# yc015/fully-automated-multi-heartbeat-echocardiography-video-segmentation-and-motion-tracking

Hardware: AMD Instinct MI355X
Metric: 32f×112×112 clips/sec at 1/2/4/8 MI355X; Dice Δ vs CPU ref (higher is better)
Workload: dtype fp32

## Files before the change

### fully-automated-multi-heartbeat-echocardiography-video-segmentation-and-motion-tracking_amd/csrc/wino4_common.h

```cpp
#pragma once
#include "common.h"

typedef float f32x2 __attribute__((ext_vector_type(2)));

struct W4Geo {
  int TR, TC;
  int TH, TW;
  int RP;
  int SS;
  int RS;
  int NI;
  int n_cob;
  int gpr;
  FastDiv fd_cob, fd_gpr, fd_th, fd_tc, fd_rp, fd_ss;
#ifdef CLASFV_KNOCKOUTS
  int stagger, stagger_groups;
#endif
};

namespace {

constexpr int W4_WAVES = 4;
constexpr int W4_THREADS = 64 * W4_WAVES;
constexpr int W4_NU = 14;
template <int DPW>
struct W4Ring {
  static constexpr int STAGE = W4_WAVES * DPW * 1024;
  static constexpr int NR = DPW == 4 ? 4 : 3;
  static constexpr int STEP = NR - 2;
  static constexpr int LDS = NR * STAGE + 1024;
};
constexpr int W4_CS = 20;
constexpr int W4_ZS = 16 * W4_CS + 4;
constexpr int W4_ZBYTES = 42 * W4_ZS * 4;
static_assert(W4_ZBYTES <= W4Ring<4>::LDS && W4Ring<4>::LDS <= 80 * 1024 && W4Ring<5>::LDS <= 80 * 1024 &&
                  W4Ring<6>::LDS <= 80 * 1024,
              "two blocks per CU");

__device__ inline int xcd_swizzle4(int b, int nb) {
  const int q = nb >> 3, r = nb & 7, x = b & 7, i = b >> 3;
  return (x < r ? x * (q + 1) : r * (q + 1) + (x - r) * q) + i;
}

constexpr int vm_wait(int n) { return (n & 0xF) | ((n >> 4) << 14) | 0x0F70; }


template <int RH>
__device__ inline void bt_rows(const f32x2 (&e)[5], f32x2 (&t)[3]) {
  if constexpr (RH == 0) {
    t[0] = e[0] * 4.f - e[2] * 5.f + e[4];
    const f32x2 s = e[1] + e[2], u = e[3] + e[4], d = e[1] - e[2], w = e[4] - e[3];
    t[1] = u - s * 4.f;
    t[2] = w + d * 4.f;
  } else {
    const f32x2 x = e[3] - e[1], y = e[2] - e[0];
    t[0] = x + y * 2.f;
    t[1] = x - y * 2.f;
    t[2] = e[0] * 4.f - e[2] * 5.f + e[4];
  }
}

template <int CH>
__device__ inline void bt_cols(const f32x2 (&t)[6], f32x2 (&v)[3]) {
  if constexpr (CH == 0) {
    v[0] = t[0] * 4.f - t[2] * 5.f + t[4];
    const f32x2 s = t[1] + t[2], u = t[3] + t[4], d = t[1] - t[2], w = t[4] - t[3];
    v[1] = u - s * 4.f;
    v[2] = w + d * 4.f;
  } else {
    const f32x2 x = t[4] - t[2], y = t[3] - t[1];
    v[0] = x + y * 2.f;
    v[1] = x - y * 2.f;
    v[2] = t[1] * 4.f - t[3] * 5.f + t[5];
  }
}

inline bool wino4_geometry(const ConvParams& p, W4Geo* g, int* n_blocks, int cob_w = 48, int fill16 = 0) {
#ifdef CLASFV_KNOCKOUTS
  g->stagger = 0;
  g->stagger_groups = 1;
#endif
  if (p.Cout % cob_w || p.Cin % 8) return false;
  const int TH = (p.Ho + 3) / 4, TW = (p.Wo + 3) / 4;
  const long rows = (long)p.N * p.To * TH;
  auto tr_for = [&](int tc) {
    for (int d = 16 / tc; d >= 1; --d)
      if (((long)p.To * TH) % d == 0) return d;
    return 1;
  };
  auto pitch = [&](int TR, int TC) {
    const int PC = 4 * TC + 2, rp0 = (PC - 1) + (PC - 1) / 4 + 1;
    int best = 1 << 30;
    for (int rp = rp0; rp < rp0 + 16; ++rp)
      for (int ss = 6 * rp; ss < 6 * rp + 16; ++ss) {
        const int ni = (2 * TR * ss + 63) / 64;
        if (ni > W4_WAVES * 6) continue;
        int cnt[16] = {0}, m = 0;
        for (int t = 0; t < TR * TC; ++t) {
          const int v = ((t / TC) * ss + 5 * (t % TC)) & 15;
          if (++cnt[v] > m) m = cnt[v];
        }
        const int score = m * 1000 + (ni <= 16 ? 0 : 100) + ni;
        if (score < best) best = score, g->RP = rp, g->SS = ss;
      }
    return best != (1 << 30);
  };
  int TC = 0;
  for (int d = TW < 16 ? TW : 16; d >= 1 && !TC; --d)
    if (TW % d == 0) TC = d;
  int TR = tr_for(TC);
  if (fill16) {
    int bc = TC, br = TR;
    for (int d = TW < 16 ? TW : 16; d >= fill16; --d)
      if (TW % d == 0 && tr_for(d) * d > br * bc) bc = d, br = tr_for(d);
    if ((bc != TC || br != TR) && br * bc >= 12 && pitch(br, bc)) TC = bc, TR = br;
  }
  if (TR * TC < 12 || !pitch(TR, TC)) return false;
  g->TR = TR, g->TC = TC, g->TH = TH, g->TW = TW;
  g->RS = TR * g->SS;
  g->NI = (2 * g->RS + 63) / 64;
  g->n_cob = p.Cout / cob_w;
  g->gpr = TW / TC;
  g->fd_cob = fast_div(g->n_cob);
  g->fd_gpr = fast_div(g->gpr);
  g->fd_th = fast_div(TH);
  g->fd_tc = fast_div(TC);
  g->fd_rp = fast_div(g->RP);
  g->fd_ss = fast_div(g->SS);
  *n_blocks = (int)(rows / TR) * g->gpr * g->n_cob;
  return true;
}

}
```

### fully-automated-multi-heartbeat-echocardiography-video-segmentation-and-motion-tracking_amd/csrc/winograd4w.hip

```cpp
#include <cstdio>
#include <cstdlib>
#include <type_traits>

#include "wino4_common.h"

namespace {

template <int NTN>
struct W4W {
  static constexpr int NV = 18 * NTN;
  static constexpr int UQ = NTN == 9 ? 14 : 9;
  static constexpr int NU = (NV + 4 * UQ - 1) / (4 * UQ) * UQ;
};

constexpr int W4W_ZT = 20;
constexpr int W4W_ZP = 16 * W4W_ZT + 4;
constexpr int W4W_ZBUF = 42 * W4W_ZP;

constexpr int W4W_NTA = 7;
__device__ inline void mfma_v(f32x4& c, float a, float b) {
  asm volatile("s_nop 1\n\tv_mfma_f32_16x16x4_f32 %0, %1, %2, %0" : "+v"(c) : "v"(a), "v"(b));
}
__device__ inline void w4w_drain() { asm volatile("s_nop 7\n\ts_nop 4" ::: "memory"); }

// ... 166 lines not shown
      if constexpr ((KO & 2) == 0) {
        const int gn = gi + UQ;
        u[gi % UQ] = gn < NU ? load_u(k, gn) : load_u(k + 1, gn - NU);
      }
    }
    constexpr int NB = (NTN < W4W_NTA ? NTN : W4W_NTA) * 18, FG = NB / 4, RM = NB % 4;
#pragma unroll
    for (int gi = 0; gi < NU; ++gi) {
      if (gi < FG)
        __builtin_amdgcn_sched_group_barrier(0x008, 4, 0);
      else if (gi == FG && RM)
        __builtin_amdgcn_sched_group_barrier(0x008, RM, 0);
      if constexpr ((KO & 2) == 0) __builtin_amdgcn_sched_group_barrier(0x020, 1, 0);
    }
  } while (++k < nchunk);
  if constexpr (NTN > W4W_NTA) w4w_drain();
  __builtin_amdgcn_s_waitcnt(vm_wait(0));
  __syncthreads();
#ifdef CLASFV_KNOCKOUTS
  if constexpr ((KO & 512) != 0) st_[2] = __builtin_amdgcn_s_memrealtime();
#endif

  if constexpr ((KO & 4) != 0) {
    float sum = 0.f;
#pragma unroll
    for (int nt = 0; nt < NTN; ++nt)
#pragma unroll
      for (int r = 0; r < 3; ++r)
#pragma unroll
        for (int jj = 0; jj < 3; ++jj) sum += acc[nt][r][jj][0] + acc[nt][r][jj][3];
    if (sum == 1234.5f) reinterpret_cast<float*>(p.y)[tid] = sum;
    return;
  }
  float* Z0 = reinterpret_cast<float*>(smem);
  const int q = lane >> 4, l16 = lane & 15;
  const size_t plane = (size_t)p.N * p.To * H * W * 8;
  float* yout = reinterpret_cast<float*>(p.y);
  const int ub = tid & 3, ucq = (tid >> 2) & 3, utile = tid >> 4;
  const int useg = fdiv(utile, g.fd_tc), utc = utile - useg * g.TC;
  const int uR = R0 + useg, uf = fdiv(uR, g.fd_th), uty = uR - uf * g.TH;
  const int uxx = 4 * (tx0 + utc) + ub;
  const bool ulive = utile < NT && uxx < W;
  const int eb = ub == 3 ? 1 : ub;
  const int CO = p.Cout;
  auto write_planes = [&](int nt) __attribute__((always_inline)) {
    float* Z = Z0 + (nt & 1) * W4W_ZBUF;
    if (ch == 0) {
#pragma unroll
      for (int r = 0; r < 3; ++r) {
        const f32x4 m0 = acc[nt][r][0], m1 = acc[nt][r][1], m2 = acc[nt][r][2];
        f32x4* zp = reinterpret_cast<f32x4*>(Z + ((3 * rh + r) * 3) * W4W_ZP + l16 * W4W_ZT + 4 * q);
        zp[0] = m0 + m1 + m2;
        zp[W4W_ZP / 4] = psub4(m1, m2);
        zp[2 * W4W_ZP / 4] = m1 + m2;
      }
    } else {
#pragma unroll
      for (int r = 0; r < 3; ++r) {
        const f32x4 m0 = acc[nt][r][0], m1 = acc[nt][r][1], m2 = acc[nt][r][2];
        f32x4* zp = reinterpret_cast<f32x4*>(Z + (18 + (3 * rh + r) * 4) * W4W_ZP + l16 * W4W_ZT + 4 * q);
        const f32x4 sm = m0 + m1, df = psub4(m0, m1);
        zp[0] = sm;
        zp[W4W_ZP / 4] = 2.f * df;
        zp[2 * W4W_ZP / 4] = 4.f * sm;
        zp[3 * W4W_ZP / 4] = 8.f * df + m2;
      }
    }
  };
  auto read_unit = [&](int nt, f32x4 (&P)[6]) __attribute__((always_inline)) {
    const float* Z = Z0 + (nt & 1) * W4W_ZBUF;
#pragma unroll
    for (int i = 0; i < 6; ++i)
      P[i] = *reinterpret_cast<const f32x4*>(Z + (i * 3 + eb) * W4W_ZP + utile * W4W_ZT + 4 * ucq) +
             *reinterpret_cast<const f32x4*>(Z + (18 + i * 4 + ub) * W4W_ZP + utile * W4W_ZT + 4 * ucq);
  };
  const int co0 = cob * NTN * 16 + 4 * ucq;
  const size_t upix = (size_t)(uf * H + 4 * uty) * W + uxx;
  float* ybase[4];
#pragma unroll
  for (int aa = 0; aa < 4; ++aa) {
    const size_t px = upix + (size_t)aa * W;
    ybase[aa] = yout + (C8 ? (size_t)(co0 >> 3) * plane + px * 8 + (co0 & 7) : px * CO + co0);
  }
  const size_t nt_step = C8 ? 2 * plane : 16;
  f32x4 biasv[NTN];
#pragma unroll
  for (int nt = 0; nt < NTN; ++nt)
    biasv[nt] = p.bias ? *reinterpret_cast<const f32x4*>(p.bias + co0 + nt * 16) : f32x4{0.f, 0.f, 0.f, 0.f};
  auto store_unit = [&](int nt, const f32x4 (&P)[6]) __attribute__((always_inline)) {
    const f32x4 bias = biasv[nt];
    const f32x4 s12 = P[1] + P[2], d12 = psub4(P[1], P[2]), s34 = P[3] + P[4], d34 = psub4(P[3], P[4]);
    f32x4 y[4];
    y[0] = P[0] + s12 + s34;
    y[1] = d12 + 2.f * d34;
    y[2] = s12 + 4.f * s34;
    y[3] = d12 + 8.f * d34 + P[5];
#pragma unroll
    for (int aa = 0; aa < 4; ++aa) {
      if (4 * uty + aa >= H) break;
      f32x4 o = y[aa] + bias;
      if constexpr (RELU) {
#pragma unroll
        for (int c = 0; c < 4; ++c) o[c] = relu1(o[c]);
      }
      float* dst = ybase[aa] + nt * nt_step;
      if constexpr ((KO & 128) != 0) {
        if (o[0] == 1234.5f) *reinterpret_cast<f32x4*>(dst) = o;
      } else {
        *reinterpret_cast<f32x4*>(dst) = o;
      }
    }
  };
  if constexpr ((KO & 256) != 0) {
#pragma unroll
    for (int nt = 0; nt < NTN; ++nt) {
      __builtin_amdgcn_sched_barrier(0);
      write_planes(nt);
      __syncthreads();
      if (ulive) {
        f32x4 P[6];
        read_unit(nt, P);
        store_unit(nt, P);
      }
    }
  } else {
    write_planes(0);
#pragma unroll
    for (int nt = 0; nt < NTN; ++nt) {
      __builtin_amdgcn_sched_barrier(0);
      __syncthreads();
      f32x4 P[6];
      if (ulive) read_unit(nt, P);
      if (nt + 1 < NTN) write_planes(nt + 1);
      if (ulive) store_unit(nt, P);
    }
  }
#ifdef CLASFV_KNOCKOUTS
  if constexpr ((KO & 512) != 0) {
    __builtin_amdgcn_s_waitcnt(0);
    __syncthreads();
    st_[3] = __builtin_amdgcn_s_memrealtime();
    if (tid == 0 && blockIdx.x < W4W_NSTAMP) {
      unsigned long long* o = g_w4w_stamps[blockIdx.x];
      o[0] = st_[0], o[1] = st_[1], o[2] = st_[2], o[3] = st_[3];
      o[8] = __builtin_amdgcn_s_getreg((4 << 0) | (0 << 6) | (31 << 11));
      o[9] = __builtin_amdgcn_s_getreg((20 << 0) | (0 << 6) | (31 << 11));
    }
  }
#endif
}

constexpr int W4R_WAVES = 12;
constexpr int W4R_THREADS = 64 * W4R_WAVES;
constexpr int W4R_DPW = 2;
constexpr int W4R_STAGE = W4R_WAVES * W4R_DPW * 1024;
constexpr int W4R_NR = 4;
constexpr int W4R_NZ = 3;
constexpr int W4R_LDS = W4R_NZ * W4W_ZBUF * 4;
static_assert(W4R_LDS >= W4R_NR * W4R_STAGE + 1024 && W4R_LDS <= 160 * 1024, "ring and planes fit LDS");

template <int NTN>
struct W4R {
  static constexpr int NV = 6 * NTN;
  static constexpr int UQ = NTN == 9 ? 7 : NTN == 5 ? 8 : 9;
  static constexpr int NU = (NV + 4 * UQ - 1) / (4 * UQ) * UQ;
};

template <int RH, int R>
__device__ inline f32x2 bt_row(const f32x2 (&e)[5]) {
  if constexpr (RH == 0) {
    if constexpr (R == 0) {
      return e[0] * 4.f - e[2] * 5.f + e[4];
    } else if constexpr (R == 1) {
      const f32x2 s = e[1] + e[2], u = e[3] + e[4];
      return u - s * 4.f;
    } else {
      const f32x2 d = e[1] - e[2], w = e[4] - e[3];
      return w + d * 4.f;
    }
  } else {
    if constexpr (R == 2) {
      return e[0] * 4.f - e[2] * 5.f + e[4];
    } else {
      const f32x2 x = e[3] - e[1], y = e[2] - e[0];
      if constexpr (R == 0)
        return x + y * 2.f;
      else
        return x - y * 2.f;
    }
  }
}

template <int NTN, bool C8, int KO = 0, bool RELU = true, int NR = W4R_NR, int CPB = 1, bool NTS = false>
__global__ __launch_bounds__(W4R_THREADS) __attribute__((amdgpu_waves_per_eu(3, 3))) void conv_wino4r(ConvParams p,
                                                                                                       W4Geo g) {
  using WR = W4R<NTN>;
  constexpr int STAGE = W4R_STAGE, UQ = WR::UQ, NU = WR::NU, NV = WR::NV;
  constexpr int STEP = NR / 2;
  static_assert(NR * STAGE + 1024 <= W4R_LDS, "ring fits the plane buffers' LDS");
  __shared__ __align__(16) char smem[W4R_LDS];
  char* sink = smem + NR * STAGE;

#ifdef CLASFV_KNOCKOUTS
  unsigned long long st_[4] = {0, 0, 0, 0};
  if constexpr ((KO & 512) != 0) st_[0] = __builtin_amdgcn_s_memrealtime();
#endif
#ifdef CLASFV_KNOCKOUTS
  if (g.stagger > 0 && blockIdx.x < 256) {
    const int sg = (blockIdx.x >> 3) % g.stagger_groups;
    if (sg) {
      const unsigned long long t0 = __builtin_amdgcn_s_memrealtime(), dt = (unsigned long long)sg * g.stagger;
      while (__builtin_amdgcn_s_memrealtime() - t0 < dt) __builtin_amdgcn_s_sleep(8);
    }
  }
#endif
  const __amdgpu_buffer_rsrc_t xr = __builtin_amdgcn_make_buffer_rsrc(
      const_cast<void*>(p.x), (short)0, (int)((size_t)p.N * p.Ti * p.Hi * p.Wi * p.Cin * 4), 0x00020000);
  const int tid = threadIdx.x, lane = tid & 63;
  const int wid = __builtin_amdgcn_readfirstlane(tid >> 6);
  const int blk = xcd_swizzle4(blockIdx.x, gridDim.x);
  const int grp = fdiv(blk, g.fd_cob), cob = blk - grp * g.n_cob;
  const int rg = fdiv(grp, g.fd_gpr), gx = grp - rg * g.gpr;
  const int R0 = rg * g.TR, tx0 = gx * g.TC;
  const int H = p.Ho, W = p.Wo, C = p.Cin;
  const int nchunk = C >> 3;
  const int NT = g.TR * g.TC;
  const int wq = wid / 3, r = wid - 3 * wq, rh = wq >> 1, ch = wq & 1;

  unsigned d_off[W4R_DPW];
#pragma unroll
  for (int j = 0; j < W4R_DPW; ++j) {
    const int ins = wid + W4R_WAVES * j, s = ins * 64 + lane;
    unsigned off = 0x80000000u;
    if (ins < g.NI && s < 2 * g.RS) {
      const int hf = s >= g.RS ? 1 : 0, sl = s - hf * g.RS;
      const int seg = fdiv(sl, g.fd_ss), ss = sl - seg * g.SS;
      const int rr = fdiv(ss, g.fd_rp), cs = ss - rr * g.RP;
      const int m5 = cs / 5, k5 = cs - 5 * m5, c = 4 * m5 + k5;
      if (rr < 6 && k5 < 4 && c < 4 * g.TC + 2) {
        const int R = R0 + seg, f = fdiv(R, g.fd_th), ty = R - f * g.TH;
        const int yy = 4 * ty - 1 + rr, xx = 4 * tx0 - 1 + c;
        if ((unsigned)yy < (unsigned)H && (unsigned)xx < (unsigned)W) off = (((f * H + yy) * W + xx) * C + hf * 4) * 4;
      }
    }
    d_off[j] = off;
  }
  auto issue_raw = [&](int k, int stage) __attribute__((always_inline)) {
#pragma unroll
    for (int j = 0; j < W4R_DPW; ++j) {
      const int ins = wid + W4R_WAVES * j;
      __builtin_amdgcn_raw_ptr_buffer_load_lds(
          xr, (__attribute__((address_space(3))) void*)(ins < g.NI ? smem + stage * STAGE + ins * 1024 : sink), 16,
          d_off[j], k < nchunk ? k * 32 : 0, 0, 0);
    }
  };

  const int t = lane & 15, k4 = lane >> 4;
  const int tv = t < NT ? t : 0;
  const int tseg = fdiv(tv, g.fd_tc), tcol = tv - tseg * g.TC;
  const int lane_off = ((k4 >> 1) * g.RS + tseg * g.SS + rh * g.RP + 5 * tcol) * 16 + (k4 & 1) * 8;
  const int rp16 = g.RP * 16;
  auto transform = [&](int stage, f32x2 (&a)[3]) __attribute__((always_inline)) {
    if constexpr ((KO & 1) != 0) {
#pragma unroll
      for (int jj = 0; jj < 3; ++jj) a[jj] = f32x2{(float)(lane + jj + stage), (float)(lane - jj)};
      return;
    }
    const char* base = smem + stage * STAGE + lane_off;
    auto body = [&](auto rh_c, auto ch_c, auto r_c) __attribute__((always_inline)) {
      constexpr int RH = decltype(rh_c)::value, CH = decltype(ch_c)::value, RR = decltype(r_c)::value;
      f32x2 tt[6];
      if constexpr (CPB == 0) {
        auto col_read = [&](int c, f32x2 (&e)[5]) __attribute__((always_inline)) {
          const int co = (c + (c >> 2)) * 16;
#pragma unroll
          for (int q = 0; q < 5; ++q) e[q] = *reinterpret_cast<const f32x2*>(base + q * rp16 + co);
        };
        f32x2 e0[5], e1[5];
        col_read(0, e0);
        __builtin_amdgcn_sched_barrier(0);
#pragma unroll
        for (int c = 0; c < 6; c += 2) {
          if (c + 1 < 6) col_read(c + 1, e1);
          tt[c] = bt_row<RH, RR>(e0);
          __builtin_amdgcn_sched_barrier(0);
          if (c + 2 < 6) col_read(c + 2, e0);
          tt[c + 1] = bt_row<RH, RR>(e1);
          __builtin_amdgcn_sched_barrier(0);
        }
      } else {
#pragma unroll
        for (int c = 0; c < 6; ++c) {
          const int co = (c + (c >> 2)) * 16;
          f32x2 e[5];
#pragma unroll
          for (int q = 0; q < 5; ++q) e[q] = *reinterpret_cast<const f32x2*>(base + q * rp16 + co);
          tt[c] = bt_row<RH, RR>(e);
          if (c % CPB == CPB - 1) __builtin_amdgcn_sched_barrier(0);
        }
      }
      bt_cols<CH>(tt, a);
    };
    using I0 = std::integral_constant<int, 0>;
    using I1 = std::integral_constant<int, 1>;
    using I2 = std::integral_constant<int, 2>;
    switch (wid) {
      case 0: body(I0{}, I0{}, I0{}); break;
      case 1: body(I0{}, I0{}, I1{}); break;
      case 2: body(I0{}, I0{}, I2{}); break;
      case 3: body(I0{}, I1{}, I0{}); break;
      case 4: body(I0{}, I1{}, I1{}); break;
      case 5: body(I0{}, I1{}, I2{}); break;
      case 6: body(I1{}, I0{}, I0{}); break;
      case 7: body(I1{}, I0{}, I1{}); break;
      case 8: body(I1{}, I0{}, I2{}); break;
      case 9: body(I1{}, I1{}, I0{}); break;
      case 10: body(I1{}, I1{}, I1{}); break;
      default: body(I1{}, I1{}, I2{}); break;
    }
  };

  const __amdgpu_buffer_rsrc_t ur = __builtin_amdgcn_make_buffer_rsrc(
      const_cast<float*>(reinterpret_cast<const float*>(p.w) + ((size_t)cob * nchunk * W4R_WAVES + wid) * (NU * 256)),
      (short)0, nchunk * W4R_WAVES * NU * 256 * 4, 0x00020000);
  auto load_u = [&](int k, int gi) __attribute__((always_inline)) {
    return __builtin_bit_cast(f32x4, __builtin_amdgcn_raw_buffer_load_b128(
                                         ur, lane * 16, ((k < nchunk ? k : 0) * (W4R_WAVES * NU * 256) + gi * 256) * 4, 0));
  };

  f32x4 acc[NTN][3];
#pragma unroll
  for (int nt = 0; nt < NTN; ++nt)
#pragma unroll
    for (int jj = 0; jj < 3; ++jj) acc[nt][jj] = f32x4{0.f, 0.f, 0.f, 0.f};
  f32x4 u[UQ];
  f32x2 a[3];

#pragma unroll
  for (int d = 0; d < STEP; ++d) {
    issue_raw(d, d);
    __builtin_amdgcn_sched_barrier(0);
  }
#pragma unroll
  for (int gi = 0; gi < UQ; ++gi) u[gi] = load_u(0, gi);
  __builtin_amdgcn_sched_barrier(0);

  int k = 0;
#pragma unroll 1
  do {
    const int ph = k % NR;
    if (ph % STEP == 0) {
      __builtin_amdgcn_s_waitcnt(vm_wait(UQ));
      __builtin_amdgcn_sched_barrier(0);
      if constexpr ((KO & 16) == 0) __builtin_amdgcn_s_barrier();
      __builtin_amdgcn_sched_barrier(0);
#ifdef CLASFV_KNOCKOUTS
      if constexpr ((KO & 512) != 0)
        if (k == 0) st_[1] = __builtin_amdgcn_s_memrealtime();
#endif
      if constexpr ((KO & 8) == 0) {
#pragma unroll
        for (int d = NR - STEP; d < NR; ++d) issue_raw(k + d, (ph + d) % NR);
      }
    }
    __builtin_amdgcn_sched_barrier(0);
    transform(ph, a);
    __builtin_amdgcn_sched_barrier(0);
#pragma unroll
    for (int gi = 0; gi < NU; ++gi) {
#pragma unroll
      for (int c = 0; c < 4; ++c) {
        const int m = 4 * gi + c;
        if (m < NV) {
          const int jj = m % 3, ks = (m / 3) % 2, nt = m / 6;
          acc[nt][jj] = __builtin_amdgcn_mfma_f32_16x16x4f32(u[gi % UQ][c], ks ? a[jj].y : a[jj].x, acc[nt][jj], 0, 0, 0);
        }
      }
      if constexpr ((KO & 2) == 0) {
        const int gn = gi + UQ;
        u[gi % UQ] = gn < NU ? load_u(k, gn) : load_u(k + 1, gn - NU);
      }
    }
    constexpr int FG = NV / 4, RM = NV % 4;
#pragma unroll
    for (int gi = 0; gi < NU; ++gi) {
      if (gi < FG)
        __builtin_amdgcn_sched_group_barrier(0x008, 4, 0);
      else if (gi == FG && RM)
        __builtin_amdgcn_sched_group_barrier(0x008, RM, 0);
      if constexpr ((KO & 2) == 0) __builtin_amdgcn_sched_group_barrier(0x020, 1, 0);
    }
  } while (++k < nchunk);
  __builtin_amdgcn_s_waitcnt(vm_wait(0));
  __syncthreads();
#ifdef CLASFV_KNOCKOUTS
  if constexpr ((KO & 512) != 0) st_[2] = __builtin_amdgcn_s_memrealtime();
#endif

  if constexpr ((KO & 4) != 0) {
    float sum = 0.f;
#pragma unroll
    for (int nt = 0; nt < NTN; ++nt)
#pragma unroll
      for (int jj = 0; jj < 3; ++jj) sum += acc[nt][jj][0] + acc[nt][jj][3];
    if (sum == 1234.5f) reinterpret_cast<float*>(p.y)[tid] = sum;
    return;
  }
  float* Z0 = reinterpret_cast<float*>(smem);
  const int q = lane >> 4, l16 = lane & 15;
  const size_t plane = (size_t)p.N * p.To * H * W * 8;
  float* yout = reinterpret_cast<float*>(p.y);
  const int ug = tid >> 8, ut = tid & 255;
  const int ub = ut & 3, ucq = (ut >> 2) & 3, utile = ut >> 4;
  const int useg = fdiv(utile, g.fd_tc), utc = utile - useg * g.TC;
  const int uR = R0 + useg, uf = fdiv(uR, g.fd_th), uty = uR - uf * g.TH;
  const int uxx = 4 * (tx0 + utc) + ub;
  const bool ulive = utile < NT && uxx < W;
  const int eb = ub == 3 ? 1 : ub;
  const int CO = p.Cout;
  const int zrow = 3 * rh + r;
  auto write_planes = [&](int nt, int buf) __attribute__((always_inline)) {
    float* Z = Z0 + buf * W4W_ZBUF;
    const f32x4 m0 = acc[nt][0], m1 = acc[nt][1], m2 = acc[nt][2];
    if (ch == 0) {
      f32x4* zp = reinterpret_cast<f32x4*>(Z + (zrow * 3) * W4W_ZP + l16 * W4W_ZT + 4 * q);
      zp[0] = m0 + m1 + m2;
      zp[W4W_ZP / 4] = psub4(m1, m2);
      zp[2 * W4W_ZP / 4] = m1 + m2;
    } else {
      f32x4* zp = reinterpret_cast<f32x4*>(Z + (18 + zrow * 4) * W4W_ZP + l16 * W4W_ZT + 4 * q);
      const f32x4 sm = m0 + m1, df = psub4(m0, m1);
      zp[0] = sm;
      zp[W4W_ZP / 4] = 2.f * df;
      zp[2 * W4W_ZP / 4] = 4.f * sm;
      zp[3 * W4W_ZP / 4] = 8.f * df + m2;
    }
  };
  auto read_unit = [&](int buf, f32x4 (&P)[6]) __attribute__((always_inline)) {
    const float* Z = Z0 + buf * W4W_ZBUF;
#pragma unroll
    for (int i = 0; i < 6; ++i)
      P[i] = *reinterpret_cast<const f32x4*>(Z + (i * 3 + eb) * W4W_ZP + utile * W4W_ZT + 4 * ucq) +
             *reinterpret_cast<const f32x4*>(Z + (18 + i * 4 + ub) * W4W_ZP + utile * W4W_ZT + 4 * ucq);
  };
  const int co0 = cob * NTN * 16 + 4 * ucq;
  const size_t upix = (size_t)(uf * H + 4 * uty) * W + uxx;
  float* ybase[4];
#pragma unroll
  for (int aa = 0; aa < 4; ++aa) {
    const size_t px = upix + (size_t)aa * W;
    ybase[aa] = yout + (C8 ? (size_t)(co0 >> 3) * plane + px * 8 + (co0 & 7) : px * CO + co0);
  }
  const size_t nt_step = C8 ? 2 * plane : 16;
  constexpr int NRND = (NTN + W4R_NZ - 1) / W4R_NZ;
  f32x4 biasv[NRND];
#pragma unroll
  for (int rd = 0; rd < NRND; ++rd) {
    const int nt = W4R_NZ * rd + ug;
    biasv[rd] = p.bias && nt < NTN ? *reinterpret_cast<const f32x4*>(p.bias + co0 + nt * 16) : f32x4{0.f, 0.f, 0.f, 0.f};
  }
  auto store_unit = [&](int nt, const f32x4& bias, const f32x4 (&P)[6]) __attribute__((always_inline)) {
    const f32x4 s12 = P[1] + P[2], d12 = psub4(P[1], P[2]), s34 = P[3] + P[4], d34 = psub4(P[3], P[4]);
    f32x4 y[4];
    y[0] = P[0] + s12 + s34;
    y[1] = d12 + 2.f * d34;
    y[2] = s12 + 4.f * s34;
    y[3] = d12 + 8.f * d34 + P[5];
#pragma unroll
    for (int aa = 0; aa < 4; ++aa) {
      if (4 * uty + aa >= H) break;
      f32x4 o = y[aa] + bias;
      if constexpr (RELU) {
#pragma unroll
        for (int c = 0; c < 4; ++c) o[c] = relu1(o[c]);
      }
      float* dst = ybase[aa] + nt * nt_step;
      if constexpr ((KO & 128) != 0) {
        if (o[0] == 1234.5f) *reinterpret_cast<f32x4*>(dst) = o;
      } else if constexpr (NTS || (KO & 2048) != 0) {
        __builtin_nontemporal_store(o, reinterpret_cast<f32x4*>(dst));
      } else {
        *reinterpret_cast<f32x4*>(dst) = o;
      }
    }
  };
#pragma unroll
  for (int b = 0; b < W4R_NZ; ++b)
    if (b < NTN) write_planes(b, b);
#pragma unroll
  for (int rd = 0; rd < NRND; ++rd) {
    __builtin_amdgcn_sched_barrier(0);
    __syncthreads();
    const int nt_u = W4R_NZ * rd + ug;
    const bool live = ulive && nt_u < NTN;
    f32x4 P[6];
    if (live) read_unit(ug, P);
    if (rd + 1 < NRND) {
      __syncthreads();
#pragma unroll
      for (int b = 0; b < W4R_NZ; ++b)
        if (W4R_NZ * (rd + 1) + b < NTN) write_planes(W4R_NZ * (rd + 1) + b, b);
    }
    if (live) store_unit(nt_u, biasv[rd], P);
  }
#ifdef CLASFV_KNOCKOUTS
  if constexpr ((KO & 512) != 0) {
    __builtin_amdgcn_s_waitcnt(0);
    __syncthreads();
    st_[3] = __builtin_amdgcn_s_memrealtime();
    if (tid == 0 && blockIdx.x < W4W_NSTAMP) {
      unsigned long long* o = g_w4w_stamps[blockIdx.x];
      o[0] = st_[0], o[1] = st_[1], o[2] = st_[2], o[3] = st_[3];
      o[8] = __builtin_amdgcn_s_getreg((4 << 0) | (0 << 6) | (31 << 11));
      o[9] = __builtin_amdgcn_s_getreg((20 << 0) | (0 << 6) | (31 << 11));
    }
  }
#endif
}

template <int NTN, int KO = 0, int NR = W4R_NR, int CPB = 1>
hipError_t launch_w4r(const ConvParams& p, const W4Geo& g, int n_blocks, hipStream_t s) {
  const dim3 grid(n_blocks), block(W4R_THREADS);
  if (!(p.vflags & CLASFV_VARIANT_W4R_CACHED_STORES)) {
    if (p.y_c8 && p.relu) {
      CLASFV_LAUNCH((conv_wino4r<NTN, true, KO, true, NR, CPB, true>), grid, block, 0, s, p, g);
      return hipGetLastError();
    }
    if (p.relu) {
      CLASFV_LAUNCH((conv_wino4r<NTN, false, KO, true, NR, CPB, true>), grid, block, 0, s, p, g);
      return hipGetLastError();
    }
  }
  if (p.y_c8 && p.relu)
    CLASFV_LAUNCH((conv_wino4r<NTN, true, KO, true, NR, CPB>), grid, block, 0, s, p, g);
  else if (p.relu)
    CLASFV_LAUNCH((conv_wino4r<NTN, false, KO, true, NR, CPB>), grid, block, 0, s, p, g);
  else if (p.y_c8)
    CLASFV_LAUNCH((conv_wino4r<NTN, true, KO, false, NR, CPB>), grid, block, 0, s, p, g);
  else
    CLASFV_LAUNCH((conv_wino4r<NTN, false, KO, false, NR, CPB>), grid, block, 0, s, p, g);
  return hipGetLastError();
}

constexpr int W4W_FILL = 1;

int wino4w_ntn(int cout) {
  if (cout % 16) return 0;
  for (int n : {9, 6})
    if ((cout / 16) % n == 0) return n;
  return 0;
}

template <int NTN, int DPW, int KO = 0>
hipError_t launch_w4w(const ConvParams& p, const W4Geo& g, int n_blocks, hipStream_t s) {
  const dim3 grid(n_blocks), block(W4_THREADS);
  if (p.y_c8 && p.relu)
    CLASFV_LAUNCH((conv_wino4w<NTN, true, DPW, KO, true>), grid, block, 0, s, p, g);
  else if (p.relu)
    CLASFV_LAUNCH((conv_wino4w<NTN, false, DPW, KO, true>), grid, block, 0, s, p, g);
  else if (p.y_c8)
    CLASFV_LAUNCH((conv_wino4w<NTN, true, DPW, KO, false>), grid, block, 0, s, p, g);
  else
    CLASFV_LAUNCH((conv_wino4w<NTN, false, DPW, KO, false>), grid, block, 0, s, p, g);
  return hipGetLastError();
}

template <int NTN, int KO = 0>
hipError_t launch_w4w_dpw(const ConvParams& p, const W4Geo& g, int n_blocks, hipStream_t s) {
  const int dpw = (g.NI + W4_WAVES - 1) / W4_WAVES;
  return dpw <= 4 ? launch_w4w<NTN, 4, KO>(p, g, n_blocks, s)
                  : dpw == 5 ? launch_w4w<NTN, 5, KO>(p, g, n_blocks, s) : launch_w4w<NTN, 6, KO>(p, g, n_blocks, s);
}

}

bool wino4w_supported(const ConvParams& p) {
  W4Geo g;
  int nb;
  const int ntn = wino4w_ntn(p.Cout);
  return ntn && !p.in_bf16 && !p.out_bf16 && !p.stem && !p.x2 && !p.res && p.KT == 1 && p.KH == 3 && p.KW == 3 &&
         p.sh == 1 && p.sw == 1 && p.st == 1 && p.ph == 1 && p.pw == 1 && p.pt == 0 && p.Ho == p.Hi &&
         p.Wo == p.Wi && p.To == p.Ti &&
         (size_t)p.N * p.To * p.Ho * p.Wo * (p.Cin > p.Cout ? p.Cin : p.Cout) < ((size_t)1 << 31) &&
         wino4_geometry(p, &g, &nb, 16 * ntn, W4W_FILL);
}

hipError_t launch_wino4w(const ConvParams& p, hipStream_t s) {
  if (!wino4w_supported(p)) return hipErrorInvalidValue;
  W4Geo g;
  int nb;
  const int ntn = wino4w_ntn(p.Cout);
  wino4_geometry(p, &g, &nb, 16 * ntn, W4W_FILL);
  return ntn == 9 ? launch_w4w_dpw<9>(p, g, nb, s) : launch_w4w_dpw<6>(p, g, nb, s);
}

double wino4w_exec_gflop(const ConvParams& p) {
  W4Geo g;
  int nb;
  const int ntn = wino4w_ntn(p.Cout);
  return ntn && wino4_geometry(p, &g, &nb, 16 * ntn, W4W_FILL) ? 2.0 * nb * 16.0 * 36.0 * p.Cin * 16.0 * ntn * 1e-9 : 0.0;
}

size_t wino4w_weight_floats(int cin_p, int cout_p) {
  const int ntn = wino4w_ntn(cout_p);
  if (!ntn) return 0;
  const int nu = ntn == 9 ? W4W<9>::NU : W4W<6>::NU;
  return (size_t)(cout_p / (16 * ntn)) * (cin_p / 8) * W4_WAVES * nu * 256;
}

void wino4w_transform_weights(const double* w, int cout, int cin, int cout_p, int cin_p, float* U) {
  static const double G[6][3] = {{1.0 / 4, 0, 0},
                                 {-1.0 / 6, -1.0 / 6, -1.0 / 6},
                                 {-1.0 / 6, 1.0 / 6, -1.0 / 6},
                                 {1.0 / 24, 1.0 / 12, 1.0 / 6},
                                 {1.0 / 24, -1.0 / 12, 1.0 / 6},
                                 {0, 0, 1}};
  const int ntn = wino4w_ntn(cout_p);
  const int nu = ntn == 9 ? W4W<9>::NU : W4W<6>::NU;
  const int nch = cin_p / 8, cw = 16 * ntn;
  const size_t total = wino4w_weight_floats(cin_p, cout_p);
  for (size_t i = 0; i < total; ++i) U[i] = 0.f;
  for (int o = 0; o < cout; ++o)
    for (int c = 0; c < cin; ++c) {
      const double* gw = w + ((size_t)o * cin + c) * 9;
      double tmp[6][3];
      for (int i = 0; i < 6; ++i)
        for (int v = 0; v < 3; ++v) tmp[i][v] = G[i][0] * gw[0 * 3 + v] + G[i][1] * gw[1 * 3 + v] + G[i][2] * gw[2 * 3 + v];
      const int cob = o / cw, nt = (o % cw) / 16, n = o % 16;
      const int chunk = c / 8, k4 = (c % 8) / 2, ks = c % 2;
      for (int i = 0; i < 6; ++i)
        for (int j = 0; j < 6; ++j) {
          const double uu = tmp[i][0] * G[j][0] + tmp[i][1] * G[j][1] + tmp[i][2] * G[j][2];
          const int wv = (i / 3) * 2 + j / 3, r = i % 3, jj = j % 3;
          const int m = ((nt * 3 + r) * 2 + ks) * 3 + jj, gi = m / 4, comp = m % 4;
          U[((((((size_t)cob * nch + chunk) * W4_WAVES + wv) * nu + gi) * 64) + k4 * 16 + n) * 4 + comp] = (float)uu;
        }
    }
}

int wino4r_ntn(int cout) {
  if (cout % 16) return 0;
  for (int n : {9, 6})
    if ((cout / 16) % n == 0) return n;
  return 0;
}

static int w4r_nu(int ntn) { return ntn == 9 ? W4R<9>::NU : ntn == 6 ? W4R<6>::NU : W4R<5>::NU; }

bool wino4r_supported(const ConvParams& p) {
  W4Geo g;
  int nb;
  const int ntn = wino4r_ntn(p.Cout);
  return ntn && !p.in_bf16 && !p.out_bf16 && !p.stem && !p.x2 && !p.res && p.KT == 1 && p.KH == 3 && p.KW == 3 &&
         p.sh == 1 && p.sw == 1 && p.st == 1 && p.ph == 1 && p.pw == 1 && p.pt == 0 && p.Ho == p.Hi &&
         p.Wo == p.Wi && p.To == p.Ti &&
         (size_t)p.N * p.To * p.Ho * p.Wo * (p.Cin > p.Cout ? p.Cin : p.Cout) < ((size_t)1 << 31) &&
         wino4_geometry(p, &g, &nb, 16 * ntn, W4W_FILL);
}

hipError_t launch_wino4r(const ConvParams& p, hipStream_t s) {
  if (!wino4r_supported(p)) return hipErrorInvalidValue;
  W4Geo g;
  int nb;
  const int ntn = wino4r_ntn(p.Cout);
  wino4_geometry(p, &g, &nb, 16 * ntn, W4W_FILL);
  return ntn == 9 ? launch_w4r<9>(p, g, nb, s) : launch_w4r<6>(p, g, nb, s);
}

double wino4r_exec_gflop(const ConvParams& p) {
  W4Geo g;
  int nb;
  const int ntn = wino4r_ntn(p.Cout);
  return ntn && wino4_geometry(p, &g, &nb, 16 * ntn, W4W_FILL) ? 2.0 * nb * 16.0 * 36.0 * p.Cin * 16.0 * ntn * 1e-9 : 0.0;
}

size_t wino4r_weight_floats(int cin_p, int cout_p) {
  const int ntn = wino4r_ntn(cout_p);
  if (!ntn) return 0;
  return (size_t)(cout_p / (16 * ntn)) * (cin_p / 8) * W4R_WAVES * w4r_nu(ntn) * 256;
}

void wino4r_transform_weights(const double* w, int cout, int cin, int cout_p, int cin_p, float* U) {
  static const double G[6][3] = {{1.0 / 4, 0, 0},
                                 {-1.0 / 6, -1.0 / 6, -1.0 / 6},
                                 {-1.0 / 6, 1.0 / 6, -1.0 / 6},
                                 {1.0 / 24, 1.0 / 12, 1.0 / 6},
                                 {1.0 / 24, -1.0 / 12, 1.0 / 6},
                                 {0, 0, 1}};
  const int ntn = wino4r_ntn(cout_p);
  const int nu = w4r_nu(ntn);
  const int nch = cin_p / 8, cw = 16 * ntn;
  const size_t total = wino4r_weight_floats(cin_p, cout_p);
  for (size_t i = 0; i < total; ++i) U[i] = 0.f;
  for (int o = 0; o < cout; ++o)
    for (int c = 0; c < cin; ++c) {
      const double* gw = w + ((size_t)o * cin + c) * 9;
      double tmp[6][3];
      for (int i = 0; i < 6; ++i)
        for (int v = 0; v < 3; ++v) tmp[i][v] = G[i][0] * gw[0 * 3 + v] + G[i][1] * gw[1 * 3 + v] + G[i][2] * gw[2 * 3 + v];
      const int cob = o / cw, nt = (o % cw) / 16, n = o % 16;
      const int chunk = c / 8, k4 = (c % 8) / 2, ks = c % 2;
      for (int i = 0; i < 6; ++i)
        for (int j = 0; j < 6; ++j) {
          const double uu = tmp[i][0] * G[j][0] + tmp[i][1] * G[j][1] + tmp[i][2] * G[j][2];
          const int wv = ((i / 3) * 2 + j / 3) * 3 + i % 3, jj = j % 3;
          const int m = (nt * 2 + ks) * 3 + jj, gi = m / 4, comp = m % 4;
          U[((((((size_t)cob * nch + chunk) * W4R_WAVES + wv) * nu + gi) * 64) + k4 * 16 + n) * 4 + comp] = (float)uu;
        }
    }
}

#ifdef CLASFV_KNOCKOUTS
void wino4w_stamps(unsigned long long* out, int n) {
  (void)hipMemcpyFromSymbol(out, HIP_SYMBOL(g_w4w_stamps), sizeof(unsigned long long) * 10 * (n < W4W_NSTAMP ? n : W4W_NSTAMP));
}
hipError_t launch_wino4w_ko(const ConvParams& p, hipStream_t s, int ko) {
  if (!wino4w_supported(p) || wino4w_ntn(p.Cout) != 9) return hipErrorInvalidValue;
  W4Geo g;
  int nb;
  wino4_geometry(p, &g, &nb, 144, (ko & 1024) ? 0 : (ko & 2048) ? 1 : W4W_FILL);
  ko &= ~3072;
  switch (ko) {
    case 1: return launch_w4w_dpw<9, 1>(p, g, nb, s);
    case 2: return launch_w4w_dpw<9, 2>(p, g, nb, s);
    case 4: return launch_w4w_dpw<9, 4>(p, g, nb, s);
    case 8: return launch_w4w_dpw<9, 8>(p, g, nb, s);
    case 15: return launch_w4w_dpw<9, 15>(p, g, nb, s);
    case 128: return launch_w4w_dpw<9, 128>(p, g, nb, s);
    case 256: return launch_w4w_dpw<9, 256>(p, g, nb, s);
    case 512: return launch_w4w_dpw<9, 512>(p, g, nb, s);
    default: return launch_w4w_dpw<9>(p, g, nb, s);
  }
}
hipError_t launch_wino4r_ko(const ConvParams& p, hipStream_t s, int ko) {
  if (!wino4w_supported(p) || wino4w_ntn(p.Cout) != 9) return hipErrorInvalidValue;
  W4Geo g;
  int nb;
  wino4_geometry(p, &g, &nb, 144, W4W_FILL);
  if (const char* e = getenv("CB_W4R_STAGGER")) sscanf(e, "%d,%d", &g.stagger, &g.stagger_groups);
  switch (ko) {
    case 1: return launch_w4r<9, 1>(p, g, nb, s);
    case 2: return launch_w4r<9, 2>(p, g, nb, s);
    case 8: return launch_w4r<9, 8>(p, g, nb, s);
    case 16: return launch_w4r<9, 16>(p, g, nb, s);
    case 31: return launch_w4r<9, 31>(p, g, nb, s);
    case 4: return launch_w4r<9, 4>(p, g, nb, s);
    case 128: return launch_w4r<9, 128>(p, g, nb, s);
    case 512: return launch_w4r<9, 512>(p, g, nb, s);
    case 64: return launch_w4r<9, 0, 6>(p, g, nb, s);
    case 32: return launch_w4r<9, 0, 4, 2>(p, g, nb, s);
    case 96: return launch_w4r<9, 0, 4, 3>(p, g, nb, s);
    case 160: return launch_w4r<9, 0, 4, 0>(p, g, nb, s);
    case 2048: return launch_w4r<9, 2048>(p, g, nb, s);
    case 576: return launch_w4r<9, 512, 6>(p, g, nb, s);
    default: return launch_w4r<9>(p, g, nb, s);
  }
}
void wino4r_from_wino4w(const float* Uw, int cin_p, int cout_p, float* Ur) {
  const int ntn = wino4w_ntn(cout_p);
  const int nuw = ntn == 9 ? W4W<9>::NU : W4W<6>::NU, nur = ntn == 9 ? W4R<9>::NU : W4R<6>::NU;
  const int nch = cin_p / 8, ncob = cout_p / (16 * ntn);
  for (size_t i = 0; i < wino4r_weight_floats(cin_p, cout_p); ++i) Ur[i] = 0.f;
  for (int cob = 0; cob < ncob; ++cob)
    for (int ck = 0; ck < nch; ++ck)
      for (int wv = 0; wv < 4; ++wv)
        for (int r = 0; r < 3; ++r)
          for (int nt = 0; nt < ntn; ++nt)
            for (int ks = 0; ks < 2; ++ks)
              for (int jj = 0; jj < 3; ++jj) {
                const int mw = ((nt * 3 + r) * 2 + ks) * 3 + jj, mr = (nt * 2 + ks) * 3 + jj;
                for (int l = 0; l < 64; ++l)
                  Ur[(((((size_t)cob * nch + ck) * W4R_WAVES + wv * 3 + r) * nur + mr / 4) * 64 + l) * 4 + mr % 4] =
                      Uw[(((((size_t)cob * nch + ck) * 4 + wv) * nuw + mw / 4) * 64 + l) * 4 + mw % 4];
              }
}
#endif
```

Measured before the change: 1448.

## Stage 32-channel input slabs per load in Winograd-4 raw kernel with double buffering

Reworks the conv_wino4r input staging so that each LDS stage holds 32 channels (8 parts of 4 channels) per pixel, using a new padded layout (LRP/LSS pitch with stride 33). Four 8-channel chunks are now transformed from each stage, and the ring becomes two buffers. This cuts the number of barrier/issue rounds and gives larger, more contiguous buffer_load_lds transfers. In exchange it needs more loads per wave, dynamic stage sizing, and an LDS-fit guard that can reject some shapes. It also turns on launch staggering for large grids by default.

```diff
diff --git a/fully-automated-multi-heartbeat-echocardiography-video-segmentation-and-motion-tracking_amd/csrc/wino4_common.h b/fully-automated-multi-heartbeat-echocardiography-video-segmentation-and-motion-tracking_amd/csrc/wino4_common.h
--- a/fully-automated-multi-heartbeat-echocardiography-video-segmentation-and-motion-tracking_amd/csrc/wino4_common.h
+++ b/fully-automated-multi-heartbeat-echocardiography-video-segmentation-and-motion-tracking_amd/csrc/wino4_common.h
@@ -13,9 +13,12 @@
   int n_cob;
   int gpr;
   FastDiv fd_cob, fd_gpr, fd_th, fd_tc, fd_rp, fd_ss;
-#ifdef CLASFV_KNOCKOUTS
+  int LRP;
+  int LSS;
+  int LSL;
+  int LNI;
+  FastDiv fd_lrp, fd_lss;
   int stagger, stagger_groups;
-#endif
 };
 
 namespace {
@@ -76,10 +79,8 @@
 }
 
 inline bool wino4_geometry(const ConvParams& p, W4Geo* g, int* n_blocks, int cob_w = 48, int fill16 = 0) {
-#ifdef CLASFV_KNOCKOUTS
   g->stagger = 0;
   g->stagger_groups = 1;
-#endif
   if (p.Cout % cob_w || p.Cin % 8) return false;
   const int TH = (p.Ho + 3) / 4, TW = (p.Wo + 3) / 4;
   const long rows = (long)p.N * p.To * TH;
@@ -127,6 +128,16 @@
   g->fd_tc = fast_div(TC);
   g->fd_rp = fast_div(g->RP);
   g->fd_ss = fast_div(g->SS);
+  g->LRP = 8 * (4 * TC + 2) + TC;
+  for (g->LSS = 6 * g->LRP;; ++g->LSS) {
+    unsigned seen = 0;
+    for (int t = 0; t < TR * TC; ++t) seen |= 1u << (((t / TC) * g->LSS + 33 * (t % TC)) & 15);
+    if (__builtin_popcount(seen) == TR * TC) break;
+  }
+  g->LSL = (TR - 1) * g->LSS + 6 * g->LRP;
+  g->LNI = (g->LSL + 63) / 64;
+  g->fd_lrp = fast_div(g->LRP);
+  g->fd_lss = fast_div(g->LSS);
   *n_blocks = (int)(rows / TR) * g->gpr * g->n_cob;
   return true;
 }
diff --git a/fully-automated-multi-heartbeat-echocardiography-video-segmentation-and-motion-tracking_amd/csrc/winograd4w.hip b/fully-automated-multi-heartbeat-echocardiography-video-segmentation-and-motion-tracking_amd/csrc/winograd4w.hip
--- a/fully-automated-multi-heartbeat-echocardiography-video-segmentation-and-motion-tracking_amd/csrc/winograd4w.hip
+++ b/fully-automated-multi-heartbeat-echocardiography-video-segmentation-and-motion-tracking_amd/csrc/winograd4w.hip
@@ -342,12 +342,12 @@
 
 constexpr int W4R_WAVES = 12;
 constexpr int W4R_THREADS = 64 * W4R_WAVES;
-constexpr int W4R_DPW = 2;
-constexpr int W4R_STAGE = W4R_WAVES * W4R_DPW * 1024;
-constexpr int W4R_NR = 4;
+constexpr int W4R_DPW = 7;
+constexpr int W4R_NR = 2;
 constexpr int W4R_NZ = 3;
 constexpr int W4R_LDS = W4R_NZ * W4W_ZBUF * 4;
-static_assert(W4R_LDS >= W4R_NR * W4R_STAGE + 1024 && W4R_LDS <= 160 * 1024, "ring and planes fit LDS");
+constexpr int W4R_MAX_LNI = (W4R_LDS - 1024) / (W4R_NR * 1024);
+static_assert(W4R_MAX_LNI <= W4R_WAVES * W4R_DPW && W4R_LDS <= 160 * 1024, "ring and planes fit LDS");
 
 template <int NTN>
 struct W4R {
@@ -381,21 +381,19 @@
   }
 }
 
-template <int NTN, bool C8, int KO = 0, bool RELU = true, int NR = W4R_NR, int CPB = 1, bool NTS = false>
+template <int NTN, bool C8, int KO = 0, bool RELU = true, int CPB = 1, bool NTS = false>
 __global__ __launch_bounds__(W4R_THREADS) __attribute__((amdgpu_waves_per_eu(3, 3))) void conv_wino4r(ConvParams p,
                                                                                                        W4Geo g) {
   using WR = W4R<NTN>;
-  constexpr int STAGE = W4R_STAGE, UQ = WR::UQ, NU = WR::NU, NV = WR::NV;
-  constexpr int STEP = NR / 2;
-  static_assert(NR * STAGE + 1024 <= W4R_LDS, "ring fits the plane buffers' LDS");
+  constexpr int UQ = WR::UQ, NU = WR::NU, NV = WR::NV;
   __shared__ __align__(16) char smem[W4R_LDS];
-  char* sink = smem + NR * STAGE;
+  const int STAGE = g.LNI * 1024;
+  char* sink = smem + W4R_NR * STAGE;
 
 #ifdef CLASFV_KNOCKOUTS
   unsigned long long st_[4] = {0, 0, 0, 0};
   if constexpr ((KO & 512) != 0) st_[0] = __builtin_amdgcn_s_memrealtime();
 #endif
-#ifdef CLASFV_KNOCKOUTS
   if (g.stagger > 0 && blockIdx.x < 256) {
     const int sg = (blockIdx.x >> 3) % g.stagger_groups;
     if (sg) {
@@ -403,7 +401,6 @@
       while (__builtin_amdgcn_s_memrealtime() - t0 < dt) __builtin_amdgcn_s_sleep(8);
     }
   }
-#endif
   const __amdgpu_buffer_rsrc_t xr = __builtin_amdgcn_make_buffer_rsrc(
       const_cast<void*>(p.x), (short)0, (int)((size_t)p.N * p.Ti * p.Hi * p.Wi * p.Cin * 4), 0x00020000);
   const int tid = threadIdx.x, lane = tid & 63;
@@ -420,49 +417,49 @@
   unsigned d_off[W4R_DPW];
 #pragma unroll
   for (int j = 0; j < W4R_DPW; ++j) {
-    const int ins = wid + W4R_WAVES * j, s = ins * 64 + lane;
+    const int s = (wid + W4R_WAVES * j) * 64 + lane;
     unsigned off = 0x80000000u;
-    if (ins < g.NI && s < 2 * g.RS) {
-      const int hf = s >= g.RS ? 1 : 0, sl = s - hf * g.RS;
-      const int seg = fdiv(sl, g.fd_ss), ss = sl - seg * g.SS;
-      const int rr = fdiv(ss, g.fd_rp), cs = ss - rr * g.RP;
-      const int m5 = cs / 5, k5 = cs - 5 * m5, c = 4 * m5 + k5;
-      if (rr < 6 && k5 < 4 && c < 4 * g.TC + 2) {
+    if (s < g.LSL) {
+      const int seg = fdiv(s, g.fd_lss), ss = s - seg * g.LSS;
+      const int rr = fdiv(ss, g.fd_lrp), cs = ss - rr * g.LRP;
+      const int m33 = cs / 33, q33 = cs - 33 * m33, c = 4 * m33 + (q33 >> 3), part = q33 & 7;
+      if (rr < 6 && q33 < 32 && c < 4 * g.TC + 2 && 4 * part < C) {
         const int R = R0 + seg, f = fdiv(R, g.fd_th), ty = R - f * g.TH;
         const int yy = 4 * ty - 1 + rr, xx = 4 * tx0 - 1 + c;
-        if ((unsigned)yy < (unsigned)H && (unsigned)xx < (unsigned)W) off = (((f * H + yy) * W + xx) * C + hf * 4) * 4;
+        if ((unsigned)yy < (unsigned)H && (unsigned)xx < (unsigned)W) off = (((f * H + yy) * W + xx) * C + 4 * part) * 4;
       }
     }
     d_off[j] = off;
   }
-  auto issue_raw = [&](int k, int stage) __attribute__((always_inline)) {
+  auto issue_raw = [&](int S, int buf) __attribute__((always_inline)) {
+    const bool live = 32 * S < C;
 #pragma unroll
     for (int j = 0; j < W4R_DPW; ++j) {
       const int ins = wid + W4R_WAVES * j;
       __builtin_amdgcn_raw_ptr_buffer_load_lds(
-          xr, (__attribute__((address_space(3))) void*)(ins < g.NI ? smem + stage * STAGE + ins * 1024 : sink), 16,
-          d_off[j], k < nchunk ? k * 32 : 0, 0, 0);
+          xr, (__attribute__((address_space(3))) void*)(ins < g.LNI ? smem + buf * STAGE + ins * 1024 : sink), 16,
+          live ? d_off[j] + 128u * S : 0x80000000u, 0, 0, 0);
     }
   };
 
   const int t = lane & 15, k4 = lane >> 4;
   const int tv = t < NT ? t : 0;
   const int tseg = fdiv(tv, g.fd_tc), tcol = tv - tseg * g.TC;
-  const int lane_off = ((k4 >> 1) * g.RS + tseg * g.SS + rh * g.RP + 5 * tcol) * 16 + (k4 & 1) * 8;
-  const int rp16 = g.RP * 16;
-  auto transform = [&](int stage, f32x2 (&a)[3]) __attribute__((always_inline)) {
+  const int lane_off = (tseg * g.LSS + rh * g.LRP + 33 * tcol) * 16 + k4 * 8;
+  const int rp16 = g.LRP * 16;
+  auto transform = [&](int buf, int kc, f32x2 (&a)[3]) __attribute__((always_inline)) {
     if constexpr ((KO & 1) != 0) {
 #pragma unroll
-      for (int jj = 0; jj < 3; ++jj) a[jj] = f32x2{(float)(lane + jj + stage), (float)(lane - jj)};
+      for (int jj = 0; jj < 3; ++jj) a[jj] = f32x2{(float)(lane + jj + buf + kc), (float)(lane - jj)};
       return;
     }
-    const char* base = smem + stage * STAGE + lane_off;
+    const char* base = smem + buf * STAGE + kc * 32 + lane_off;
     auto body = [&](auto rh_c, auto ch_c, auto r_c) __attribute__((always_inline)) {
       constexpr int RH = decltype(rh_c)::value, CH = decltype(ch_c)::value, RR = decltype(r_c)::value;
       f32x2 tt[6];
       if constexpr (CPB == 0) {
         auto col_read = [&](int c, f32x2 (&e)[5]) __attribute__((always_inline)) {
-          const int co = (c + (c >> 2)) * 16;
+          const int co = (8 * c + (c >> 2)) * 16;
 #pragma unroll
           for (int q = 0; q < 5; ++q) e[q] = *reinterpret_cast<const f32x2*>(base + q * rp16 + co);
         };
@@ -481,7 +478,7 @@
       } else {
 #pragma unroll
         for (int c = 0; c < 6; ++c) {
-          const int co = (c + (c >> 2)) * 16;
+          const int co = (8 * c + (c >> 2)) * 16;
           f32x2 e[5];
 #pragma unroll
           for (int q = 0; q < 5; ++q) e[q] = *reinterpret_cast<const f32x2*>(base + q * rp16 + co);
@@ -527,34 +524,37 @@
   f32x2 a[3];
 
 #pragma unroll
-  for (int d = 0; d < STEP; ++d) {
+  for (int d = 0; d < W4R_NR; ++d) {
     issue_raw(d, d);
     __builtin_amdgcn_sched_barrier(0);
   }
 #pragma unroll
   for (int gi = 0; gi < UQ; ++gi) u[gi] = load_u(0, gi);
   __builtin_amdgcn_sched_barrier(0);
+  static_assert(W4R_DPW + UQ <= 63, "vmcnt field");
+  __builtin_amdgcn_s_waitcnt(vm_wait(W4R_DPW + UQ));
+  __builtin_amdgcn_sched_barrier(0);
+  if constexpr ((KO & 16) == 0) __builtin_amdgcn_s_barrier();
+  __builtin_amdgcn_sched_barrier(0);
+#ifdef CLASFV_KNOCKOUTS
+  if constexpr ((KO & 512) != 0) st_[1] = __builtin_amdgcn_s_memrealtime();
+#endif
 
   int k = 0;
 #pragma unroll 1
   do {
-    const int ph = k % NR;
-    if (ph % STEP == 0) {
+    const int kc = k & 3, S = k >> 2, buf = S & 1;
+    if (kc == 0 && k > 0) {
       __builtin_amdgcn_s_waitcnt(vm_wait(UQ));
       __builtin_amdgcn_sched_barrier(0);
       if constexpr ((KO & 16) == 0) __builtin_amdgcn_s_barrier();
       __builtin_amdgcn_sched_barrier(0);
-#ifdef CLASFV_KNOCKOUTS
-      if constexpr ((KO & 512) != 0)
-        if (k == 0) st_[1] = __builtin_amdgcn_s_memrealtime();
-#endif
       if constexpr ((KO & 8) == 0) {
-#pragma unroll
-        for (int d = NR - STEP; d < NR; ++d) issue_raw(k + d, (ph + d) % NR);
+        if (32 * (S + 1) < C) issue_raw(S + 1, buf ^ 1);
       }
     }
     __builtin_amdgcn_sched_barrier(0);
-    transform(ph, a);
+    transform(buf, kc, a);
     __builtin_amdgcn_sched_barrier(0);
 #pragma unroll
     for (int gi = 0; gi < NU; ++gi) {
@@ -708,27 +708,27 @@
 #endif
 }
 
-template <int NTN, int KO = 0, int NR = W4R_NR, int CPB = 1>
+template <int NTN, int KO = 0, int CPB = 1>
 hipError_t launch_w4r(const ConvParams& p, const W4Geo& g, int n_blocks, hipStream_t s) {
   const dim3 grid(n_blocks), block(W4R_THREADS);
   if (!(p.vflags & CLASFV_VARIANT_W4R_CACHED_STORES)) {
     if (p.y_c8 && p.relu) {
-      CLASFV_LAUNCH((conv_wino4r<NTN, true, KO, true, NR, CPB, true>), grid, block, 0, s, p, g);
+      CLASFV_LAUNCH((conv_wino4r<NTN, true, KO, true, CPB, true>), grid, block, 0, s, p, g);
       return hipGetLastError();
     }
     if (p.relu) {
-      CLASFV_LAUNCH((conv_wino4r<NTN, false, KO, true, NR, CPB, true>), grid, block, 0, s, p, g);
+      CLASFV_LAUNCH((conv_wino4r<NTN, false, KO, true, CPB, true>), grid, block, 0, s, p, g);
       return hipGetLastError();
     }
   }
   if (p.y_c8 && p.relu)
-    CLASFV_LAUNCH((conv_wino4r<NTN, true, KO, true, NR, CPB>), grid, block, 0, s, p, g);
+    CLASFV_LAUNCH((conv_wino4r<NTN, true, KO, true, CPB>), grid, block, 0, s, p, g);
   else if (p.relu)
-    CLASFV_LAUNCH((conv_wino4r<NTN, false, KO, true, NR, CPB>), grid, block, 0, s, p, g);
+    CLASFV_LAUNCH((conv_wino4r<NTN, false, KO, true, CPB>), grid, block, 0, s, p, g);
   else if (p.y_c8)
-    CLASFV_LAUNCH((conv_wino4r<NTN, true, KO, false, NR, CPB>), grid, block, 0, s, p, g);
+    CLASFV_LAUNCH((conv_wino4r<NTN, true, KO, false, CPB>), grid, block, 0, s, p, g);
   else
-    CLASFV_LAUNCH((conv_wino4r<NTN, false, KO, false, NR, CPB>), grid, block, 0, s, p, g);
+    CLASFV_LAUNCH((conv_wino4r<NTN, false, KO, false, CPB>), grid, block, 0, s, p, g);
   return hipGetLastError();
 }
 
@@ -845,7 +845,13 @@
          p.sh == 1 && p.sw == 1 && p.st == 1 && p.ph == 1 && p.pw == 1 && p.pt == 0 && p.Ho == p.Hi &&
          p.Wo == p.Wi && p.To == p.Ti &&
          (size_t)p.N * p.To * p.Ho * p.Wo * (p.Cin > p.Cout ? p.Cin : p.Cout) < ((size_t)1 << 31) &&
-         wino4_geometry(p, &g, &nb, 16 * ntn, W4W_FILL);
+         wino4_geometry(p, &g, &nb, 16 * ntn, W4W_FILL) && g.LNI <= W4R_MAX_LNI;
+}
+
+static void w4r_stagger(const ConvParams& p, int ntn, int n_blocks, W4Geo* g) {
+  if (n_blocks < 16 * 256) return;
+  g->stagger_groups = 8;
+  g->stagger = (1370 + 264 * (p.Cin / 8) * ntn / 9) / 8;
 }
 
 hipError_t launch_wino4r(const ConvParams& p, hipStream_t s) {
@@ -854,6 +860,7 @@
   int nb;
   const int ntn = wino4r_ntn(p.Cout);
   wino4_geometry(p, &g, &nb, 16 * ntn, W4W_FILL);
+  w4r_stagger(p, ntn, nb, &g);
   return ntn == 9 ? launch_w4r<9>(p, g, nb, s) : launch_w4r<6>(p, g, nb, s);
 }
 
@@ -937,12 +944,10 @@
     case 4: return launch_w4r<9, 4>(p, g, nb, s);
     case 128: return launch_w4r<9, 128>(p, g, nb, s);
     case 512: return launch_w4r<9, 512>(p, g, nb, s);
-    case 64: return launch_w4r<9, 0, 6>(p, g, nb, s);
-    case 32: return launch_w4r<9, 0, 4, 2>(p, g, nb, s);
-    case 96: return launch_w4r<9, 0, 4, 3>(p, g, nb, s);
-    case 160: return launch_w4r<9, 0, 4, 0>(p, g, nb, s);
+    case 32: return launch_w4r<9, 0, 2>(p, g, nb, s);
+    case 96: return launch_w4r<9, 0, 3>(p, g, nb, s);
+    case 160: return launch_w4r<9, 0, 0>(p, g, nb, s);
     case 2048: return launch_w4r<9, 2048>(p, g, nb, s);
-    case 576: return launch_w4r<9, 512, 6>(p, g, nb, s);
     default: return launch_w4r<9>(p, g, nb, s);
   }
 }
```

Result: faster. 1464 (median of 6 runs) (+1.1%).
